# pacellie/raytracer_challenge

Measured on AMD Instinct MI355X. Metric: Mrays/s (unique rays: primary+shadow+reflection+refraction) at 1920x1080 depth-5, higher is better.
Workload: dtype f64

## Files before the change

### raytracer_challenge_amd/csrc/device_scene.h

```cpp
#pragma once
#include <stddef.h>
#include <stdint.h>

enum { OP_PRIM = 0, OP_GROUP = 1, OP_MESH = 2, OP_BVH = 3, OP_QUIRK = 4, OP_QGRID = 5, OP_CSG = 6, OP_CSG_END = 7 };

struct DOp {
  int32_t op, a, b, c;
  int32_t g;
  int32_t pad[3];
};

#define RTC_KOPS 12
#define RTC_KPLANES 6
struct DPlaneK {
  double row[4];
  int32_t prim;
  int32_t gcond;
  int32_t pad[2];
  double n[3];
};

struct DBvhNode {
  float lo0[3], hi0[3];
  float lo1[3], hi1[3];
// ... 168 lines not shown
  unsigned long long accel_nodes, group_tests, tri_tests, analytic_tests;
  unsigned long long knodes;
  unsigned long long kplanes;
  unsigned long long light_cells;
  unsigned long long kgroups;
  unsigned long long diag[64];
  unsigned long long nan_ts;
  unsigned long long guard;
  unsigned long long guard_claim;
  long long guard_info[8];
  unsigned long long wf_overflow;
};
#define RTC_STATS_LAUNCH_BYTES offsetof(DStats, nan_ts)

#define RTC_MAX_FUEL 16

#if defined(__HIPCC__) || defined(RTC_EMU)
#define RTC_HD __host__ __device__
#else
#define RTC_HD
#endif
static inline RTC_HD unsigned long long rtc_mix64(unsigned long long x) {
  x ^= x >> 33; x *= 0xff51afd7ed558ccdull; x ^= x >> 33; x *= 0xc4ceb9fe1a85ec53ull; x ^= x >> 33;
  return x;
}
static inline RTC_HD unsigned long long rtc_hit_hash_base(unsigned long long t_bits, int32_t prim, int32_t push) {
  return rtc_mix64(t_bits) ^ ((((unsigned long long)(uint32_t)prim << 32) | (unsigned long long)(uint32_t)push) * 0x9E3779B97F4A7C15ull);
}
static inline RTC_HD unsigned long long rtc_hit_hash(unsigned long long base, int depth, int kind) {
  return rtc_mix64(base ^ ((unsigned long long)(((unsigned)depth << 8) | (unsigned)kind) + 1ull) * 0xD6E8FEB86659FD93ull);
}

static inline RTC_HD unsigned long long rtc_splitmix64(unsigned long long z) {
  z = (z ^ (z >> 30)) * 0xbf58476d1ce4e5b9ull; z = (z ^ (z >> 27)) * 0x94d049bb133111ebull;
  return z ^ (z >> 31);
}
static inline RTC_HD unsigned long long rtc_area_hash(int light, double x, double y, double z) {
  unsigned long long bx, by, bz;
  __builtin_memcpy(&bx, &x, 8); __builtin_memcpy(&by, &y, 8); __builtin_memcpy(&bz, &z, 8);
  return rtc_splitmix64(rtc_splitmix64(rtc_splitmix64(rtc_splitmix64((unsigned long long)(uint32_t)light) ^ bx) ^ by) ^ bz);
}
static inline RTC_HD double rtc_area_jitter(unsigned long long h, unsigned j) {
  return (double)(rtc_splitmix64(h ^ (unsigned long long)j) >> 11) * 0x1.0p-53;
}
#define RTC_ALIGHT 16
#define RTC_SLIGHT 22

#define RTC_WF_SHADE_COUNT 32
#define RTC_WF_OVERFLOW 63
#define RTC_WF_CHUNK_NEXT 64
#define RTC_WF_TOP_COUNT (64 + 32 * 8 * (RTC_MAX_FUEL + 2))
#define RTC_WF_SHADE_TOP_COUNT (RTC_WF_TOP_COUNT + 32)
#define RTC_WF_COUNTS (RTC_WF_TOP_COUNT + 64)
#ifndef RTC_WF_CHUNK
#define RTC_WF_CHUNK 64u
#endif
#define RTC_SR_PLAIN 0x40000000
#define RTC_WF_MISS (-2)
struct DWave {
  double* rq[2];
  double* h_t;
  int32_t* h_prim;
  double* h_n12;
  double* sr;
  int32_t* sr_mat;
  int32_t* sr_node;
  double* contrib;
  int32_t* child;
  uint32_t* counts;
  uint32_t cap;
  uint32_t pad;
  unsigned long long* dig;
};
static inline uint64_t dwave_bytes(uint64_t cap, int levels) {
  return cap * (uint64_t)(7 + 7 + 1 + 2 + 9 + 3 * levels) * sizeof(double) + (cap * (uint64_t)(1 + 1 + 1 + 2 * levels) + RTC_WF_COUNTS) * sizeof(int32_t);
}
static inline void dwave_carve(DWave* W, void* mem, uint64_t cap, int levels) {
  double* d = (double*)mem;
  W->rq[0] = d; d += 7 * cap;
  W->rq[1] = d; d += 7 * cap;
  W->h_t = d; d += cap;
  W->h_n12 = d; d += 2 * cap;
  W->sr = d; d += 9 * cap;
  W->contrib = d; d += 3 * (uint64_t)levels * cap;
  int32_t* q = (int32_t*)d;
  W->h_prim = q; q += cap;
  W->sr_mat = q; q += cap;
  W->sr_node = q; q += cap;
  W->child = q; q += 2 * (uint64_t)levels * cap;
  W->counts = (uint32_t*)q;
  W->cap = (uint32_t)cap;
  W->pad = 0;
  W->dig = nullptr;
}
#ifndef RTC_BVH_STACK
#define RTC_BVH_STACK 64
#endif
```

### raytracer_challenge_amd/csrc/rtc_kernels.hip

```cpp
#include <cstdio>
#include <cstdlib>
#include <utility>

#include "../../include/rtc.h"
#include "rtc_device.hpp"

#ifdef RTC_EMU
#include "rtc_feat.hip"
constexpr int RTC_VARIANTS_BUILT = 6;
#else
constexpr int RTC_VARIANTS_BUILT = RTC_N_VARIANTS;
#endif
template <int... V>
static const RtcVariantOps& rtc_ops(int v, std::integer_sequence<int, V...>) {
  static const RtcVariantOps ops[RTC_N_VARIANTS] = {rtc_variant_ops<V>()...};
  return ops[v];
}
static const RtcVariantOps& rtc_ops(int v) { return rtc_ops(v, std::make_integer_sequence<int, RTC_VARIANTS_BUILT>{}); }
static int rtc_variant(const DScene& S, bool wavefront) {
  return rtc_pick_variant(rtc_scene_feat(S), S.n_kops > 0, S.has_area != 0, S.has_uv != 0, S.has_spot != 0, wavefront);
}

#ifndef RTC_WF_SHADE_WAVES
#define RTC_WF_SHADE_WAVES 4
// ... 138 lines not shown
    }
    if (!PIPE || n_waves != 8)
#endif
    if (threadIdx.x == 0) {
      unsigned t[4] = {0u, 0u, 0u, 0u}, b[4];
      for (int k = 0; k < 5; k++)
        for (int w = 0; w < n_waves; w++) t[end_of[k]] += s_cnt[8 * k + w];
      const int row[4] = {RTC_WF_SHADE_COUNT + level, RTC_WF_SHADE_TOP_COUNT + level, level + 1, RTC_WF_TOP_COUNT + level + 1};
      for (int e = 0; e < 4; e++) {
        const unsigned old = t[e] ? atomicAdd(&W.counts[row[e]], t[e]) : 0u;
        const bool fits = (unsigned long long)old + t[e] <= W.cap;
        if (!fits) { W.counts[RTC_WF_OVERFLOW] = 1u; stats->wf_overflow = 1ull; }
        b[e] = (e & 1) ? (fits ? W.cap - old - t[e] : W.cap) : old;
      }
      for (int k = 0; k < 5; k++)
        for (int w = 0; w < n_waves; w++) { const unsigned r = s_cnt[8 * k + w]; s_cnt[8 * k + w] = b[end_of[k]]; b[end_of[k]] += r; }
    }
    __syncthreads();
    const unsigned s = on_plane ? s_cnt[wave] + (unsigned)__popcll(m_rec0 & lt) : s_cnt[8 + wave] + (unsigned)__popcll(m_rec1 & lt);
    const unsigned jr = on_plane ? s_cnt[16 + wave] + (unsigned)__popcll(m_c0 & lt) : s_cnt[24 + wave] + (unsigned)__popcll(m_c1 & lt);
    const unsigned jt = s_cnt[32 + wave] + (unsigned)__popcll(m_c2 & lt);
    if (hit && s < W.cap) {
      double* r = W.sr;
      r[s] = st.px; r[cap + s] = st.py; r[2 * cap + s] = st.pz;
      r[3 * cap + s] = st.nx; r[4 * cap + s] = st.ny; r[5 * cap + s] = st.nz;
      if (mat >= 0) {
        r[6 * cap + s] = cr; r[7 * cap + s] = cg; r[8 * cap + s] = cbl;
        W.sr_mat[s] = mat;
      } else {
        if (!PIPE) shading_row = (int)S.mat[8 * ~mat + 7];
        W.sr_mat[s] = RTC_SR_PLAIN | shading_row;
      }
      W.sr_node[s] = (int32_t)i;
    }
    if (spawn.refl && jr < W.cap) {
      nq[jr] = st.px; nq[cap + jr] = st.py; nq[2 * cap + jr] = st.pz; nq[3 * cap + jr] = st.rx; nq[4 * cap + jr] = st.ry; nq[5 * cap + jr] = st.rz;
      nq[6 * cap + jr] = spawn.wr;
      ch[i] = (int32_t)jr;
      n_reflect++;
    }
    if (spawn.refr && jt < W.cap) {
      nq[jt] = st.ux; nq[cap + jt] = st.uy; nq[2 * cap + jt] = st.uz; nq[3 * cap + jt] = spawn.tdx; nq[4 * cap + jt] = spawn.tdy; nq[5 * cap + jt] = spawn.tdz;
      nq[6 * cap + jt] = spawn.wt;
      ch[cap + i] = (int32_t)jt;
      n_refract++;
    }
  }
  if (COUNT) {
    atomicAdd(&stats->rays_reflect, (unsigned long long)n_reflect);
    atomicAdd(&stats->rays_refract, (unsigned long long)n_refract);
  }
}

__global__ void __launch_bounds__(256) wf_gather(DCamera cam, DPixelMap pm, DWave W, unsigned n0, double* __restrict__ rgb) {
  const WorkMap wm = make_workmap(pm, cam);
  const size_t cap = W.cap;
  for (unsigned i = blockIdx.x * blockDim.x + threadIdx.x; i < n0; i += gridDim.x * blockDim.x) {
    uint64_t q;
    if (!work_to_slot(wm, i, q)) continue;
    double r = 0.0, g = 0.0, b = 0.0;
    int wait_idx[RTC_MAX_FUEL + 1];
    int wait_lvl[RTC_MAX_FUEL + 1];
    int sp = 0, lvl = 0, idx = (int)i;
    const bool digest = W.dig != nullptr && pm.digest != nullptr;
    unsigned long long dg = 0ull;
    int kind = 0;
    for (;;) {
      const double* cb = W.contrib + (size_t)lvl * 3 * cap;
      const int32_t* ch = W.child + (size_t)lvl * 2 * cap;
      const int a = ch[idx], c = ch[cap + idx];
      if (a != RTC_WF_MISS) { r += cb[idx]; g += cb[cap + idx]; b += cb[2 * cap + idx]; }
      if (digest) dg += rtc_hit_hash(W.dig[(size_t)lvl * cap + idx], lvl, kind);
      if (c >= 0) { wait_idx[sp] = c; wait_lvl[sp] = lvl + 1; sp++; }
      if (a >= 0) { idx = a; lvl++; kind = 1; continue; }
      if (sp == 0) break;
      sp--;
      idx = wait_idx[sp]; lvl = wait_lvl[sp]; kind = 2;
    }
    rgb[3 * q + 0] = r; rgb[3 * q + 1] = g; rgb[3 * q + 2] = b;
    if (digest) pm.digest[q] = dg;
  }
}


unsigned rtc_wavefront_lds_bytes(const DScene& S, bool enabled) {
#ifdef RTC_EMU
  enabled = false;
#endif
  return rtc_pick_lds_bytes(RTC_VARIANTS[rtc_variant(S, true)], enabled, rtc_lds_table_bytes(S), S.bvh_stack);
}
static RtcWfShadeBuild rtc_scene_shade_build(const DScene& S, bool count, bool level0) {
#ifdef RTC_EMU
  const bool uv = false;
#else
  const bool uv = S.has_uv != 0;
#endif
  return rtc_pick_wf_shade_build(count, uv, S.all_plain != 0, level0);
}

void rtc_kernel_info_fill(const DScene& S, bool wavefront, bool count, bool big_scene, unsigned lds_bytes, int device, rtc_kernel_info* out) {
  const int v = rtc_variant(S, wavefront);
  out->variant = v;
  out->n_kops = S.n_kops; out->n_kplanes = S.n_kplanes; out->n_kaux = 0;
  for (int i = 0; i < S.n_kops; i++) if ((S.kops[i].op == OP_BVH || S.kops[i].op == OP_MESH) && S.kops[i].pad[0] >= 0) out->n_kaux++;
  out->has_recs = S.has_recs; out->all_plain = S.all_plain; out->no_glass_mirror = S.no_glass_mirror;
  out->big_scene = big_scene ? 1 : 0;
  out->n_bvh_nodes = S.n_bvh; out->n_recs = S.n_recs; out->n_mesh_tris = S.n_mtri; out->has_mesh = S.has_mesh; out->bvh_stack = S.bvh_stack;
  out->lds_bytes = wavefront ? lds_bytes : 0u;
  out->lds_refused = 0;
#ifndef RTC_EMU
  if (wavefront && lds_bytes && rtc_ops(v).wf_ts_lds_refused && rtc_ops(v).wf_ts_lds_refused(device)) out->lds_refused = 1;
#endif
  out->trace_build = out->wf_ts_build = out->wf_shade_build0 = out->wf_shade_build = -1;
  if (wavefront) {
    out->wf_ts_build = rtc_pick_wf_ts_build(count, lds_bytes != 0);
    out->wf_shade_build0 = rtc_scene_shade_build(S, count, true);
    out->wf_shade_build = rtc_scene_shade_build(S, count, false);
  } else {
    out->trace_build = rtc_pick_trace_build(RTC_VARIANTS[v], count, big_scene, S.all_plain != 0, S.no_glass_mirror != 0);
  }
}
bool rtc_scene_is_big(unsigned long long scene_bytes) { return rtc_big_scene(scene_bytes); }

#ifndef RTC_EMU

unsigned rtc_wavefront_grid(const DScene& S, int n_cu) {
  return (unsigned)std::max(1, n_cu * rtc_ops(rtc_variant(S, true)).wf_ts_blocks_per_cu(rtc_stack_bytes(S)));
}
unsigned rtc_wavefront_lds_grid(int n_cu, int spare) { return rtc_pick_wf_ts_lds_grid(n_cu, spare); }
int rtc_wavefront_spare_cus_default(int n_cu) { return rtc_wf_spare_cus_default(n_cu); }
#endif

uint64_t rtc_wavefront_work(const DCamera& cam, const DPixelMap& pm) {
  if (pm.mode == 2 && cam.hsize >= 8 && pm.n % cam.hsize == 0) return (uint64_t)((cam.hsize + 7) / 8) * ((pm.n / cam.hsize + 7) / 8) * 64;
  return pm.n;
}

#ifndef RTC_EMU
void rtc_launch_wf_background(const DScene& S, const DCamera& cam, const DPixelMap& pm, const DWave& W, int level, unsigned n0, const DBackground& bg, unsigned blocks,
                              hipStream_t stream);
#endif
void rtc_launch_wavefront(const DScene& S, const DCamera& cam, const DPixelMap& pm, int fuel, const DWave& W, double* rgb, double* hit_t, int* hit_prim, int* hit_k,
                          DStats* stats, bool count, hipStream_t stream, unsigned blocks, unsigned shade_blocks, unsigned lds, unsigned lds_blocks, const DBackground* bg, const DBumpTable* bump) {
  if (pm.n == 0) return;
  const RtcVariantOps& ops = rtc_ops(rtc_variant(S, true));
  const RtcFrame F = {S, cam, pm, hit_t, hit_prim, hit_k, stats, stream, count};
  const unsigned n0 = (unsigned)rtc_wavefront_work(cam, pm);
  const dim3 sgrid(std::max(1u, shade_blocks)), sblock(RTC_WF_SHADE_BLOCK);
  for (int level = 0; level <= fuel + 1; level++) {
    const int tl = level <= fuel ? level : -1, sl = level - 1;
#ifndef RTC_EMU
    if (!lds || !ops.launch_wf_ts_lds(F, RtcLevel{W, tl, sl, n0, level, fuel - level, std::max(1u, lds_blocks), lds}))
#endif
    ops.launch_wf_ts(F, RtcLevel{W, tl, sl, n0, level, fuel - level, blocks, 0u});
#ifndef RTC_EMU
    if (bg && level <= fuel) rtc_launch_wf_background(S, cam, pm, W, level, n0, *bg, 4u * std::max(1u, shade_blocks), stream);
#endif
#ifndef RTC_EMU
    if (bump && level <= fuel) {
      DSceneNp N;
      static_cast<DScene&>(N) = S;
      N.bg = DBackground{0, 0};
      N.bump = *bump;
      switch (rtc_pick_wf_shade_np_build(count, S.has_uv != 0)) {
        case RTC_SH_NP_COUNT_UV: hipLaunchKernelGGL((wf_shade<true, true, true, false, false, true>), sgrid, sblock, 0, stream, N, cam, pm, W, level, n0, fuel, stats); break;
        case RTC_SH_NP_UV: hipLaunchKernelGGL((wf_shade<false, true, true, false, false, true>), sgrid, sblock, 0, stream, N, cam, pm, W, level, n0, fuel, stats); break;
        case RTC_SH_NP_COUNT: hipLaunchKernelGGL((wf_shade<true, true, false, false, false, true>), sgrid, sblock, 0, stream, N, cam, pm, W, level, n0, fuel, stats); break;
        case RTC_SH_NP: hipLaunchKernelGGL((wf_shade<false, true, false, false, false, true>), sgrid, sblock, 0, stream, N, cam, pm, W, level, n0, fuel, stats); break;
      }
    } else
#endif
    if (level <= fuel) {
      switch (rtc_scene_shade_build(S, count, level == 0)) {
#ifndef RTC_EMU
        case RTC_SH_COUNT_UV: hipLaunchKernelGGL((wf_shade<true, true, true>), sgrid, sblock, 0, stream, S, cam, pm, W, level, n0, fuel, stats); break;
        case RTC_SH_UV: hipLaunchKernelGGL((wf_shade<false, true, true>), sgrid, sblock, 0, stream, S, cam, pm, W, level, n0, fuel, stats); break;
#else
        case RTC_SH_COUNT_UV: case RTC_SH_UV: break;
#endif
        case RTC_SH_COUNT: hipLaunchKernelGGL((wf_shade<true>), sgrid, sblock, 0, stream, S, cam, pm, W, level, n0, fuel, stats); break;
        case RTC_SH_PIPE_LV0: hipLaunchKernelGGL((wf_shade<false, false, false, true, true>), sgrid, sblock, 0, stream, S, cam, pm, W, level, n0, fuel, stats); break;
        case RTC_SH_PIPE: hipLaunchKernelGGL((wf_shade<false, false, false, true, false>), sgrid, sblock, 0, stream, S, cam, pm, W, level, n0, fuel, stats); break;
        case RTC_SH_PAT: hipLaunchKernelGGL((wf_shade<false>), sgrid, sblock, 0, stream, S, cam, pm, W, level, n0, fuel, stats); break;
      }
    }
  }
  hipLaunchKernelGGL(wf_gather, dim3(std::max(1u, std::min(blocks, (n0 + 255u) / 256u))), dim3(256), 0, stream, cam, pm, W, n0, rgb);
}
void rtc_launch_wavefront(const DScene& S, const DCamera& cam, const DPixelMap& pm, int fuel, const DWave& W, double* rgb, double* hit_t, int* hit_prim, int* hit_k,
                          DStats* stats, bool count, hipStream_t stream, unsigned blocks, unsigned shade_blocks) {
  rtc_launch_wavefront(S, cam, pm, fuel, W, rgb, hit_t, hit_prim, hit_k, stats, count, stream, blocks, shade_blocks, 0u, 0u, nullptr, nullptr);
}

static dim3 rtc_elementwise_grid(unsigned long long n) { return dim3((unsigned)std::min<unsigned long long>((n + 255) / 256, 8192)); }
__global__ void __launch_bounds__(256) rtc_quantize_kernel(const double* __restrict__ rgb, unsigned char* __restrict__ out, unsigned long long n) {
  unsigned long long i = (unsigned long long)blockIdx.x * blockDim.x + threadIdx.x;
  const unsigned long long stride = (unsigned long long)gridDim.x * blockDim.x;
  for (; i < n; i += stride) {
    double x = rgb[i];
    double c = (x != x) ? 1.0 : (x < 1.0 ? x : 1.0);
    c = c > 0.0 ? c : 0.0;
    double r = round(c * 255.0);
    out[i] = (unsigned char)(r <= 0.0 ? 0.0 : (r >= 255.0 ? 255.0 : r));
  }
}
__global__ void __launch_bounds__(256) rtc_pack_hits_kernel(const double* __restrict__ t, const int* __restrict__ prim, const int* __restrict__ k, DHit* __restrict__ out, unsigned long long n) {
  for (unsigned long long i = (unsigned long long)blockIdx.x * blockDim.x + threadIdx.x; i < n; i += (unsigned long long)gridDim.x * blockDim.x) {
    DHit h;
    h.t = t[i]; h.prim = prim[i]; h.k = k[i];
    out[i] = h;
  }
}
void rtc_launch_pack_hits(const double* t, const int* prim, const int* k, DHit* out, unsigned long long n, hipStream_t stream) {
  if (n == 0) return;
  hipLaunchKernelGGL(rtc_pack_hits_kernel, rtc_elementwise_grid(n), dim3(256), 0, stream, t, prim, k, out, n);
}
void rtc_launch_quantize(const double* rgb, unsigned char* out, unsigned long long n, hipStream_t stream) {
  if (n == 0) return;
  hipLaunchKernelGGL(rtc_quantize_kernel, rtc_elementwise_grid(n), dim3(256), 0, stream, rgb, out, n);
}


template <typename T>
__global__ void __launch_bounds__(256) rtc_deinterleave_kernel(const T* __restrict__ slab, T* __restrict__ image, unsigned rowlen, unsigned vsize, unsigned n, unsigned max_rows,
                                                               unsigned band) {
  const unsigned long long total = (unsigned long long)vsize * rowlen;
  for (unsigned long long i = (unsigned long long)blockIdx.x * blockDim.x + threadIdx.x; i < total; i += (unsigned long long)gridDim.x * blockDim.x) {
    const unsigned y = (unsigned)(i / rowlen), x = (unsigned)(i % rowlen);
    const unsigned b = y / band;
    image[i] = slab[((unsigned long long)(b % n) * max_rows + (b / n) * band + y % band) * rowlen + x];
  }
}
template <typename T>
static void launch_deinterleave(const T* slab, T* image, unsigned rowlen, unsigned vsize, unsigned n, unsigned max_rows, unsigned band, hipStream_t stream) {
  const unsigned long long total = (unsigned long long)vsize * rowlen;
  if (total == 0) return;
  hipLaunchKernelGGL(rtc_deinterleave_kernel<T>, rtc_elementwise_grid(total), dim3(256), 0, stream, slab, image, rowlen, vsize, n, max_rows, band ? band : 1u);
}
void rtc_launch_deinterleave8(const unsigned char* slab, unsigned char* image, unsigned rowlen, unsigned vsize, unsigned n, unsigned max_rows, unsigned band, hipStream_t stream) {
  launch_deinterleave(slab, image, rowlen, vsize, n, max_rows, band, stream);
}
void rtc_launch_deinterleave(const double* slab, double* image, unsigned rowlen, unsigned vsize, unsigned n, unsigned max_rows, unsigned band, hipStream_t stream) {
  launch_deinterleave(slab, image, rowlen, vsize, n, max_rows, band, stream);
}
// ... 9 lines not shown
```

### raytracer_challenge_amd/csrc/rtc_scene.cpp

```cpp
#include <hip/hip_runtime_api.h>

#include <algorithm>
#include <atomic>
#include <chrono>
#include <cmath>
#include <condition_variable>
#include <cstdlib>
#include <cstdio>
#include <cstring>
#include <deque>
#include <functional>
#include <initializer_list>
#include <memory>
#include <mutex>
#include <string>
#include <thread>
#include <vector>

#include "../../include/rtc.h"
#include "adaptive_contrast.h"
#include "background_point.h"
#include "bump_normal.h"
#include "camera_sampling.h"
#include "device_scene.h"
#include "filter_weights.h"
#include "scene_build.hpp"
#include "shutter_pose.h"
#include "spot_factor.h"
#include "uv_image.h"

void rtc_launch_trace(const DScene& S, const DCamera& cam, const DPixelMap& pm, int fuel, double* rgb, double* hit_t, int* hit_prim, int* hit_k,
                      DStats* stats, bool count, hipStream_t stream, bool big_scene);
void rtc_launch_quantize(const double* rgb, unsigned char* out, unsigned long long n, hipStream_t stream);
void rtc_launch_pack_hits(const double* t, const int* prim, const int* k, DHit* out, unsigned long long n, hipStream_t stream);
void rtc_launch_deinterleave(const double* slab, double* image, unsigned rowlen, unsigned vsize, unsigned n, unsigned max_rows, unsigned band, hipStream_t stream);
void rtc_launch_deinterleave8(const unsigned char* slab, unsigned char* image, unsigned rowlen, unsigned vsize, unsigned n, unsigned max_rows, unsigned band, hipStream_t stream);
void rtc_launch_wavefront(const DScene& S, const DCamera& cam, const DPixelMap& pm, int fuel, const DWave& W, double* rgb, double* hit_t, int* hit_prim, int* hit_k,
                          DStats* stats, bool count, hipStream_t stream, unsigned blocks, unsigned shade_blocks, unsigned lds, unsigned lds_blocks, const DBackground* bg,
                          const DBumpTable* bump);
void rtc_launch_trace_np(const DScene& S, const DBumpTable& bt, const DBackground* bg, const DCamera& cam, const DPixelMap& pm, int fuel, double* rgb, double* hit_t,
                         int* hit_prim, int* hit_k, DStats* stats, bool count, hipStream_t stream);
void rtc_launch_bump_normals(const DScene& S, const DBumpTable& bt, const int32_t* prims, const double* points, const double* normals, unsigned long long n, double* out,
                             hipStream_t stream);
int rtc_bump_trace_build(const DScene& S, bool has_bg);
void rtc_launch_trace_bg(const DScene& S, const DBackground& bg, const DCamera& cam, const DPixelMap& pm, int fuel, double* rgb, double* hit_t, int* hit_prim, int* hit_k,
                         DStats* stats, bool count, hipStream_t stream);
void rtc_launch_background_colors(const DScene& S, const DBackground& bg, const double* dirs, unsigned long long n, double* rgb, hipStream_t stream);
int rtc_background_trace_build(const DScene& S);
void rtc_kernel_info_fill(const DScene& S, bool wavefront, bool count, bool big_scene, unsigned lds_bytes, int device, rtc_kernel_info* out);
bool rtc_scene_is_big(unsigned long long scene_bytes);
uint64_t rtc_wavefront_work(const DCamera& cam, const DPixelMap& pm);
unsigned rtc_wavefront_grid(const DScene& S, int n_cu);
unsigned rtc_wavefront_lds_grid(int n_cu, int spare);
int rtc_wavefront_spare_cus_default(int n_cu);
unsigned rtc_wavefront_lds_bytes(const DScene& S, bool enabled);
void rtc_launch_gen_rays(const DCamera& cam, const DPixelMap& pm, const rtc_sampling& sp, unsigned long long slot_first, unsigned long long n_slots, double* rays,
                         hipStream_t stream);
void rtc_launch_resolve_samples(const double* ray_rgb, unsigned n_samples, unsigned long long n_slots, double* dst, hipStream_t stream);
unsigned long long rtc_contrast_blocks(unsigned long long n);
unsigned long long rtc_contrast_work_words(unsigned long long n);
unsigned long long rtc_scan_work_words(unsigned long long n);
unsigned rtc_launch_scan(unsigned long long* v, unsigned long long n, unsigned long long* levels, unsigned long long* total, hipStream_t stream);
unsigned rtc_launch_contrast_compact(const double* frame, unsigned long long hsize, unsigned long long vsize, double threshold, unsigned neighbours,
                                     unsigned long long* work, unsigned long long* list, unsigned long long* count, hipStream_t stream);
void rtc_launch_resolve_samples_scatter(const double* ray_rgb, unsigned n_samples, unsigned long long n_slots, const unsigned long long* indices, double* frame,
                                        hipStream_t stream);
unsigned rtc_launch_resolve_filtered(const rtc_filter& f, const rtc_sampling& sp, unsigned long long hsize, unsigned long long row0, unsigned long long row1,
                                     unsigned long long out0, unsigned long long out1, const double* samples, double* dst, hipStream_t stream, unsigned* tile);
unsigned long long rtc_shutter_work_words(unsigned long long m);
unsigned long long* rtc_shutter_offsets(unsigned long long* work, unsigned long long m);
unsigned rtc_launch_shutter_deal(const rtc_shutter& sh, const rtc_sampling& sp, unsigned K, const DPixelMap& pm, const DCamera& cam, unsigned long long slot_first,
                                 unsigned long long m, unsigned long long* work, unsigned* order, unsigned* where, hipStream_t stream);
void rtc_launch_shutter_gen_rays(const DCamera& cam, const DPixelMap& pm, const rtc_sampling& sp, unsigned long long slot_first, const unsigned* order, unsigned off, unsigned len,
                                 unsigned m, double* rays, hipStream_t stream);
void rtc_launch_shutter_resolve(const double* ray_rgb, const unsigned* where, unsigned n_samples, unsigned long long n_slots, double* dst, hipStream_t stream);
int32_t rtc_bvh_build_device(const std::vector<bvh::Item>& items, std::vector<DBvhNode>& n2, std::vector<uint32_t>& order, uint32_t base, int leaf_max, double* frame);
int32_t rtc_bvh_build_device_keys(const std::vector<bvh::Item>& items, std::vector<DBvhNode>& n2, std::vector<uint32_t>& order, uint32_t base, int leaf_max, double* frame,
                                  std::vector<unsigned long long>* keys);

static thread_local std::string g_rtc_err;
static int rtc_fail(int code, const std::string& m) {
  g_rtc_err = m;
  return code;
}
#define HIP_OK(expr)                                                                                     \
  do {                                                                                                   \
    hipError_t e_ = (expr);                                                                              \
    if (e_ != hipSuccess) return rtc_fail(RTC_ERR_DEVICE, std::string(#expr) + ": " + hipGetErrorString(e_)); \
  } while (0)

struct rtc_scene {
  int device = 0;
// ... 3 lines not shown
  bool marker_recorded[8] = {false, false, false, false, false, false, false, false};
  std::vector<void*> allocs;
  uint64_t bytes = 0;
  DScene d{};
  bool has_bg = false;
  DBackground bg{0, 0};
  bool bg_plain = false;
  bool has_bump = false;
  uint32_t n_bumps = 0;
  DBumpTable bump{nullptr, nullptr};
  DStats* d_stats = nullptr;
  double* d_rgb = nullptr;
  double* d_hit_t = nullptr;
  int* d_hit_prim = nullptr;
  int* d_hit_k = nullptr;
  DHit* d_hits = nullptr;
  unsigned long long* d_digest = nullptr;
  unsigned long long* d_wave_dig = nullptr;
  uint64_t cap_digest = 0, cap_wave_dig = 0;
  uint8_t* d_rgb8 = nullptr;
  uint64_t cap_hits = 0, cap_rgb8 = 0;
  uint64_t* d_idx = nullptr;
  double* d_rays = nullptr;
  uint64_t cap_px = 0, cap_idx = 0, cap_rays = 0;
  double* d_srays = nullptr;
  double* d_srgb = nullptr;
  uint64_t cap_srays = 0, cap_srgb = 0;
  hipEvent_t evs0 = nullptr, evs1 = nullptr;
  unsigned long long* d_alist = nullptr;
  unsigned long long* d_awork = nullptr;
  unsigned long long* d_acount = nullptr;
  uint64_t cap_alist = 0;
  unsigned* d_shorder = nullptr;
  unsigned* d_shwhere = nullptr;
  unsigned long long* d_shwork = nullptr;
  uint64_t cap_shutter = 0;
  int kernel_version = 0;
  uint64_t tune_sig = 0;
  double tune_ms[2] = {-1.0, -1.0};
  int tune_n[2] = {0, 0};
  int tune_choice = 0;
  uint32_t n_analytic = 0;
  uint32_t n_bouncing = 0;
  uint32_t n_prims_total = 0;
  bool last_wavefront = false;
  int last_fuel = 0;
  DCsgHit* csg_slab = nullptr;
  uint64_t csg_slab_threads = 0;
  bool wave_alloc_failed = false;
  DWave wave{};
  void* wave_mem = nullptr;
  uint64_t wave_cap = 0;
  int wave_levels = 0;
  unsigned wave_blocks = 0, shade_blocks = 0;
  unsigned lds_bytes = 0;
  int n_cu = 1;
  int spare_cus = 0;
  bool counted = false;
  unsigned wave_eighths = 9;
  int bvh_depth = 0;
  int built_on_device = 0;
  uint32_t n_bvh_nodes = 0, n_mesh_tris = 0;

  template <class T>
  int upload(const std::vector<T>& v, const T** out) {
    *out = nullptr;
    if (v.empty()) return RTC_OK;
    void* p = nullptr;
    HIP_OK(hipMalloc(&p, v.size() * sizeof(T)));
    allocs.push_back(p);
    bytes += v.size() * sizeof(T);
    HIP_OK(hipMemcpy(p, v.data(), v.size() * sizeof(T), hipMemcpyHostToDevice));
    *out = (const T*)p;
    return RTC_OK;
  }
};

namespace {

struct GrowBuf { void** p; uint64_t bytes; };
int grow(uint64_t* cap, uint64_t need, std::initializer_list<GrowBuf> bufs, hipStream_t wait = nullptr) {
  if (need <= *cap) return RTC_OK;
  if (wait) HIP_OK(hipStreamSynchronize(wait));
  for (const GrowBuf& b : bufs) { (void)hipFree(*b.p); *b.p = nullptr; }
  *cap = 0;
  for (const GrowBuf& b : bufs) HIP_OK(hipMalloc(b.p, b.bytes));
  *cap = need;
  return RTC_OK;
}

int ensure_px(rtc_scene* s, uint64_t n, bool hits) {
  int rc = grow(&s->cap_px, n, {{(void**)&s->d_rgb, n * 3 * sizeof(double)}, {(void**)&s->d_hit_t, n * sizeof(double)},
                                {(void**)&s->d_hit_prim, n * sizeof(int)}, {(void**)&s->d_hit_k, n * sizeof(int)}});
  if (rc == RTC_OK && hits) rc = grow(&s->cap_hits, n, {{(void**)&s->d_hits, n * sizeof(DHit)}});
  return rc;
}
int ensure_rgb8(rtc_scene* s, uint64_t n) { return grow(&s->cap_rgb8, 3 * n, {{(void**)&s->d_rgb8, 3 * n}}); }
int ensure_rays(rtc_scene* s, uint64_t n) { return grow(&s->cap_rays, n, {{(void**)&s->d_rays, n * 6 * sizeof(double)}}); }

void pretouch_pages(void* p, size_t bytes, std::vector<std::thread>* pool) {
  if (!p || bytes < (4u << 20)) return;
  static const int T = [] { const char* e = std::getenv("RTC_PRETOUCH_THREADS"); int t = e ? std::atoi(e) : 0; return t < 0 ? 0 : (t > 32 ? 32 : t); }();
  if (T == 0) return;
  char* base = (char*)p;
  const size_t per = ((bytes / (size_t)T) + 4095) & ~(size_t)4095;
  for (int t = 0; t < T; t++) {
    const size_t b = std::min(bytes, per * (size_t)t), e = std::min(bytes, per * (size_t)(t + 1));
    if (e > b) pool->emplace_back([base, b, e] { for (size_t o = b; o < e; o += 4096) { volatile char* q = base + o; *q = 0; } });
  }
}
void join_all(std::vector<std::thread>* pool) {
  for (auto& t : *pool) t.join();
  pool->clear();
}

uint64_t wave_cap(uint64_t n_work, unsigned eighths) { return std::max<uint64_t>((n_work * eighths + 7) / 8, 4096); }
uint64_t wave_bytes(uint64_t cap, int lv) { return dwave_bytes(cap, lv); }
uint64_t wave_budget() {
  const char* e = std::getenv("RTC_WF_MAX_BYTES");
  return e ? std::strtoull(e, nullptr, 10) : (24ull << 30);
}
int ensure_wave(rtc_scene* s, uint64_t n_work, int fuel) {
  const int levels = fuel + 1;
  uint64_t cap = wave_cap(n_work, s->wave_eighths);
  if (cap > 0x7fffff00ull || wave_bytes(cap, levels) > wave_budget()) return rtc_fail(RTC_ERR_UNSUPPORTED, "launch too large for the wavefront path");
  if (cap <= s->wave_cap && levels <= s->wave_levels) return RTC_OK;
  cap = std::max(cap, s->wave_cap);
  const int lv = std::max(levels, s->wave_levels);
  HIP_OK(hipStreamSynchronize(s->stream));
  if (s->wave_mem) (void)hipFree(s->wave_mem);
  s->wave_mem = nullptr; s->wave_cap = 0; s->wave_levels = 0;
  {
    size_t free_b = 0, total_b = 0;
    if (hipMemGetInfo(&free_b, &total_b) == hipSuccess && wave_bytes(cap, lv) > (uint64_t)free_b)
      return rtc_fail(RTC_ERR_UNSUPPORTED, "the wavefront queues do not fit the device's free memory");
    const hipError_t e = std::getenv("RTC_WF_FAIL_ALLOC") ? hipErrorOutOfMemory : hipMalloc(&s->wave_mem, wave_bytes(cap, lv));
    if (e != hipSuccess) {
      (void)hipGetLastError();
      s->wave_mem = nullptr;
      if (e == hipErrorOutOfMemory) return rtc_fail(RTC_ERR_UNSUPPORTED, "hipMalloc of the wavefront queues: out of memory");
      return rtc_fail(RTC_ERR_DEVICE, std::string("hipMalloc of the wavefront queues: ") + hipGetErrorString(e));
    }
  }
  dwave_carve(&s->wave, s->wave_mem, cap, lv);
  s->wave_cap = cap;
  s->wave_levels = lv;
  return RTC_OK;
}

void to_dcam(const rtc_camera& c, DCamera* d) {
  d->hsize = c.hsize; d->vsize = c.vsize;
  d->half_width = c.half_width; d->half_height = c.half_height; d->pixel_size = c.pixel_size;
  std::memcpy(d->inv, c.transform_inv, sizeof(d->inv));
}

uint64_t launch_signature(const DCamera& cam, const DPixelMap& pm, int fuel) {
  uint64_t h = 1469598103934665603ull;
  auto mix = [&](const void* p, size_t n) { for (size_t i = 0; i < n; i++) { h ^= ((const unsigned char*)p)[i]; h *= 1099511628211ull; } };
  mix(&cam, sizeof(cam));
  mix(&pm.n, sizeof(pm.n)); mix(&pm.mode, sizeof(pm.mode)); mix(&pm.row_first, sizeof(pm.row_first)); mix(&pm.row_step, sizeof(pm.row_step)); mix(&pm.band, sizeof(pm.band));
  mix(&fuel, sizeof(fuel));
  return h ? h : 1;
}

int first_guess(const rtc_scene* s, uint64_t n_work, int fuel) {
  if (const char* e = std::getenv("RTC_FIRST_GUESS")) { const int v = std::atoi(e); if (v == 1 || v == 4) return v; }
  const bool deep = fuel >= 2 && (uint64_t)s->n_bouncing * 10u >= (uint64_t)s->n_prims_total && s->n_bouncing > 0;
  return (s->n_analytic >= 32 && deep && n_work >= (256u << 10)) ? 4 : 1;
}
int pick_path(rtc_scene* s, uint64_t sig, uint64_t n_work, int fuel, bool will_sync, bool pixel_list) {
  if (sig != s->tune_sig) { s->tune_sig = sig; s->tune_ms[0] = s->tune_ms[1] = -1.0; s->tune_n[0] = s->tune_n[1] = 0; s->tune_choice = 0; }
  if (pixel_list) return 1;
  if (s->tune_choice) return s->tune_choice;
  const int guess = first_guess(s, n_work, fuel);
  if (!will_sync) return guess;
  const int other = guess == 4 ? 1 : 4;
  const int ng = s->tune_n[guess == 4 ? 1 : 0], no = s->tune_n[other == 4 ? 1 : 0];
  return ng <= no ? guess : other;
}
void drop_wavefront(rtc_scene* s) { s->tune_ms[1] = 1e30; s->tune_n[1] = 2; s->tune_choice = 1; }
void record_sample(rtc_scene* s, bool wavefront, double ms) {
  const int k = wavefront ? 1 : 0;
  s->tune_ms[k] = s->tune_n[k] ? std::min(s->tune_ms[k], ms) : ms;
  s->tune_n[k]++;
  if (s->tune_n[0] >= 2 && s->tune_n[1] >= 2) s->tune_choice = s->tune_ms[1] < s->tune_ms[0] ? 4 : 1;
}

constexpr int RTC_LIVE_DEVICES = 64;
std::atomic<int> g_live_scenes[RTC_LIVE_DEVICES];
int live_scenes(int device) { return device >= 0 && device < RTC_LIVE_DEVICES ? g_live_scenes[device].load(std::memory_order_relaxed) : 0; }

unsigned lds_grid(const rtc_scene* s, bool will_sync) {
  const bool spare = !will_sync && live_scenes(s->device) > 1;
  return rtc_wavefront_lds_grid(s->n_cu, spare ? s->spare_cus : 0);
}

int read_clear_sticky(rtc_scene* s, DStats* h) {
  HIP_OK(hipMemcpy(h, s->d_stats, sizeof(*h), hipMemcpyDeviceToHost));
  if (h->nan_ts || h->guard || h->wf_overflow)
    HIP_OK(hipMemset((char*)s->d_stats + RTC_STATS_LAUNCH_BYTES, 0, sizeof(DStats) - RTC_STATS_LAUNCH_BYTES));
  return RTC_OK;
}

int fill_stats(rtc_scene* s, const DStats& h, uint64_t pixels, rtc_stats* stats) {
  float ms = 0.f;
  HIP_OK(hipEventElapsedTime(&ms, s->ev0, s->ev1));
  std::memset(stats, 0, sizeof(*stats));
  stats->pixels = pixels;
  stats->rays_primary = h.rays_primary; stats->rays_shadow = h.rays_shadow; stats->rays_reflect = h.rays_reflect; stats->rays_refract = h.rays_refract;
  stats->rays_container = h.rays_container; stats->accel_nodes = h.accel_nodes; stats->group_tests = h.group_tests; stats->tri_tests = h.tri_tests;
  stats->analytic_tests = h.analytic_tests; stats->nan_ts = h.nan_ts;
  stats->accel_nodes_kernarg = h.knodes; stats->analytic_tests_kernarg = h.kplanes; stats->light_grid_cells = h.light_cells;
  stats->group_tests_uniform = h.kgroups;
  stats->kernel_ms = ms;
  stats->n_launches = s->last_wavefront ? 2u * (uint32_t)s->last_fuel + 4u + (s->has_bg ? (uint32_t)s->last_fuel + 1u : 0u) : 1u;
  return RTC_OK;
}

typedef std::function<int()> AfterLaunch;
int run(rtc_scene* s, const DCamera& cam, DPixelMap pm, int fuel, double* d_rgb, bool want_hits, rtc_stats* stats, bool count, bool sync, int force = 0,
        const AfterLaunch* after = nullptr) {
  if (fuel < 0) fuel = 0;
  if (fuel > RTC_MAX_FUEL) return rtc_fail(RTC_ERR_UNSUPPORTED, "fuel exceeds RTC_MAX_FUEL (16): the reference recurses without a limit, the device keeps its pending rays per lane");
  if (s->d.n_lights == 0) fuel = 0;
  HIP_OK(hipSetDevice(s->device));
  HIP_OK(hipMemsetAsync(s->d_stats, 0, RTC_STATS_LAUNCH_BYTES, s->stream));
  HIP_OK(hipEventRecord(s->ev0, s->stream));
  const bool will_sync = sync || stats != nullptr;
  const bool tuned = force == 0 && s->kernel_version == 0;
  int path = force ? force : s->kernel_version;
  if (tuned) path = pick_path(s, launch_signature(cam, pm, fuel), rtc_wavefront_work(cam, pm), fuel, will_sync, pm.mode != 2);
  if (path == 4 && s->wave_alloc_failed && force == 0) path = 1;
  const bool wavefront = path == 4 && pm.n > 0;
  if (s->d.csg_max_hits > RTC_CSG_MAX_HITS) {
    const uint64_t threads = wavefront ? (uint64_t)s->wave_blocks * 64ull : ((rtc_wavefront_work(cam, pm) + 63) / 64) * 64;
    if (threads > s->csg_slab_threads) {
      const uint64_t bytes = threads * (uint64_t)s->d.csg_max_hits * sizeof(DCsgHit);
      const char* e = std::getenv("RTC_CSG_MAX_BYTES");
      if (bytes > (e ? std::strtoull(e, nullptr, 10) : (16ull << 30)))
        return rtc_fail(RTC_ERR_UNSUPPORTED, "the CSG intersection slab of this launch exceeds RTC_CSG_MAX_BYTES: render fewer pixels per call");
      const int rc = grow(&s->csg_slab_threads, threads, {{(void**)&s->csg_slab, bytes}}, s->stream);
      if (rc != RTC_OK) return rc;
    }
    s->d.csg_slab = s->csg_slab;
  }
  if (wavefront) {
    int rc = ensure_wave(s, rtc_wavefront_work(cam, pm), fuel);
    if (rc == RTC_ERR_UNSUPPORTED && force == 0) {
      if (tuned) drop_wavefront(s);
      else s->wave_alloc_failed = true;
      return run(s, cam, pm, fuel, d_rgb, want_hits, stats, count, sync, 1, after);
    }
    if (rc != RTC_OK) return rc;
    s->wave.dig = nullptr;
    if (pm.digest && count) {
      const uint64_t need = (uint64_t)s->wave_cap * (uint64_t)(fuel + 1);
      rc = grow(&s->cap_wave_dig, need, {{(void**)&s->d_wave_dig, need * sizeof(unsigned long long)}}, s->stream);
      if (rc != RTC_OK) return rc;
      s->wave.dig = s->d_wave_dig;
    }
    HIP_OK(hipMemsetAsync(s->wave.counts, 0, RTC_WF_COUNTS * sizeof(uint32_t), s->stream));
    HIP_OK(hipEventRecord(s->ev0, s->stream));
    rtc_launch_wavefront(s->d, cam, pm, fuel, s->wave, d_rgb, want_hits ? s->d_hit_t : nullptr, s->d_hit_prim, s->d_hit_k, s->d_stats, count, s->stream, s->wave_blocks, s->shade_blocks, s->lds_bytes,
                         lds_grid(s, will_sync), s->has_bg ? &s->bg : nullptr, s->has_bump ? &s->bump : nullptr);
  } else if (s->has_bump) {
    rtc_launch_trace_np(s->d, s->bump, s->has_bg ? &s->bg : nullptr, cam, pm, fuel, d_rgb, want_hits ? s->d_hit_t : nullptr, s->d_hit_prim, s->d_hit_k, s->d_stats, count, s->stream);
  } else if (s->has_bg) {
    rtc_launch_trace_bg(s->d, s->bg, cam, pm, fuel, d_rgb, want_hits ? s->d_hit_t : nullptr, s->d_hit_prim, s->d_hit_k, s->d_stats, count, s->stream);
  } else {
    rtc_launch_trace(s->d, cam, pm, fuel, d_rgb, want_hits ? s->d_hit_t : nullptr, s->d_hit_prim, s->d_hit_k, s->d_stats, count, s->stream, rtc_scene_is_big(s->bytes));
  }
  HIP_OK(hipGetLastError());
  HIP_OK(hipEventRecord(s->ev1, s->stream));
  s->last_wavefront = wavefront;
  s->last_fuel = fuel;
  if (after) { int rca = (*after)(); if (rca != RTC_OK) return rca; }
  if (!sync && !stats) return RTC_OK;
  HIP_OK(hipStreamSynchronize(s->stream));
  DStats h;
  int rcs = read_clear_sticky(s, &h);
  if (rcs != RTC_OK) return rcs;
  if (wavefront) {
    if (std::getenv("RTC_WF_DUMP_COUNTS")) {
      uint32_t c[64], top[64];
      HIP_OK(hipMemcpy(c, s->wave.counts, sizeof(c), hipMemcpyDeviceToHost));
      HIP_OK(hipMemcpy(top, s->wave.counts + RTC_WF_TOP_COUNT, sizeof(top), hipMemcpyDeviceToHost));
      std::fprintf(stderr, "[rtc-wf] level: rays far + near / shade records far + near:");
      for (int l = 0; l <= fuel; l++)
        std::fprintf(stderr, " %d: %u + %u / %u + %u;", l, top[l], l ? c[l] : (unsigned)rtc_wavefront_work(cam, pm), top[32 + l], c[RTC_WF_SHADE_COUNT + l]);
      std::fprintf(stderr, "\n");
    }
    uint32_t overflow = 0;
    HIP_OK(hipMemcpy(&overflow, s->wave.counts + RTC_WF_OVERFLOW, sizeof(overflow), hipMemcpyDeviceToHost));
    if (overflow) {
      const uint64_t n_work = rtc_wavefront_work(cam, pm);
      if (s->wave_eighths < 512 && wave_bytes(wave_cap(n_work, 2 * s->wave_eighths), fuel + 1) <= wave_budget() && wave_cap(n_work, 2 * s->wave_eighths) <= 0x7fffff00ull) {
        s->wave_eighths *= 2;
        const int rc2 = run(s, cam, pm, fuel, d_rgb, want_hits, stats, count, true, 4, after);
        if (rc2 != RTC_ERR_UNSUPPORTED) return rc2;
      }
      if (tuned) drop_wavefront(s);
      return run(s, cam, pm, fuel, d_rgb, want_hits, stats, count, true, 1, after);
    }
  }
  if (tuned && !count && pm.mode == 2 && !s->tune_choice) {
    float ms = 0.f;
    HIP_OK(hipEventElapsedTime(&ms, s->ev0, s->ev1));
    record_sample(s, wavefront, ms);
  }
  if (stats) {
    int rcf = fill_stats(s, h, pm.n, stats);
    if (rcf != RTC_OK) return rcf;
  }
  if (std::getenv("RTC_DIAG_DUMP")) {
    std::fprintf(stderr, "[rtc-diag]");
    for (int i = 0; i < 64; i++) std::fprintf(stderr, " %llu", (unsigned long long)h.diag[i]);
    std::fprintf(stderr, "\n");
  }
  if (h.guard) return rtc_fail(RTC_ERR_DEVICE, "traversal guard tripped (mask " + std::to_string(h.guard) + "): an index left its array; no pixel since the last check is trustworthy");
  if (h.nan_ts) return rtc_fail(RTC_ERR_NAN, "a NaN intersection t reached a sort of two or more intersections (the reference panics in Intersection::sort, src/intersection.rs:124)");
  return RTC_OK;
}

int make_pixel_map(rtc_scene* s, uint64_t hsize, uint64_t total, const uint64_t* pixel_indices, uint64_t first, uint64_t n, DPixelMap* pm, std::vector<uint64_t>* range_idx) {
  *pm = DPixelMap{};
  pm->n = n;
  if (!pixel_indices) {
    if (first % hsize == 0 && n % hsize == 0) {
      pm->mode = 2; pm->row_first = (uint32_t)(first / hsize); pm->row_step = 1;
    } else {
      range_idx->resize(n);
      for (uint64_t i = 0; i < n; i++) (*range_idx)[i] = first + i;
      pixel_indices = range_idx->data();
    }
  }
  if (pixel_indices) {
    for (uint64_t i = 0; i < n; i++)
      if (pixel_indices[i] >= total) return rtc_fail(RTC_ERR_INVALID, "pixel index exceeds the image");
    const int rc = grow(&s->cap_idx, n, {{(void**)&s->d_idx, n * sizeof(uint64_t)}});
    if (rc != RTC_OK) return rc;
    HIP_OK(hipMemcpy(s->d_idx, pixel_indices, n * sizeof(uint64_t), hipMemcpyHostToDevice));
    pm->mode = 1; pm->indices = s->d_idx;
  }
  return RTC_OK;
}
int make_pixel_map(rtc_scene* s, const rtc_camera* cam, const uint64_t* pixel_indices, uint64_t first, uint64_t n, DPixelMap* pm, std::vector<uint64_t>* range_idx) {
  return make_pixel_map(s, cam->hsize, cam->hsize * cam->vsize, pixel_indices, first, n, pm, range_idx);
}
// ... 1713 lines not shown
```

Measured before the change: 13480.

## Double-buffer wavefront counters and zero the spare set inside the gather kernel

Keeps two sets of wavefront queue counters and ping-pongs between them each frame. The final gather kernel clears the used words of the other set, so the per-frame hipMemsetAsync on the counters is usually skipped. The stats memset and the timing event records are also skipped when no sync, stats or counting is requested. This cuts stream commands between frames but adds host-side state tracking for whether each counter block is clean, which is a correctness risk if it falls out of step.

```diff
diff --git a/raytracer_challenge_amd/csrc/device_scene.h b/raytracer_challenge_amd/csrc/device_scene.h
--- a/raytracer_challenge_amd/csrc/device_scene.h
+++ b/raytracer_challenge_amd/csrc/device_scene.h
@@ -244,6 +244,7 @@
 #define RTC_WF_TOP_COUNT (64 + 32 * 8 * (RTC_MAX_FUEL + 2))
 #define RTC_WF_SHADE_TOP_COUNT (RTC_WF_TOP_COUNT + 32)
 #define RTC_WF_COUNTS (RTC_WF_TOP_COUNT + 64)
+#define RTC_WF_COUNT_BLOCKS 2
 #ifndef RTC_WF_CHUNK
 #define RTC_WF_CHUNK 64u
 #endif
@@ -265,7 +266,17 @@
   unsigned long long* dig;
 };
 static inline uint64_t dwave_bytes(uint64_t cap, int levels) {
-  return cap * (uint64_t)(7 + 7 + 1 + 2 + 9 + 3 * levels) * sizeof(double) + (cap * (uint64_t)(1 + 1 + 1 + 2 * levels) + RTC_WF_COUNTS) * sizeof(int32_t);
+  return cap * (uint64_t)(7 + 7 + 1 + 2 + 9 + 3 * levels) * sizeof(double) +
+         (cap * (uint64_t)(1 + 1 + 1 + 2 * levels) + RTC_WF_COUNT_BLOCKS * RTC_WF_COUNTS) * sizeof(int32_t);
+}
+static inline RTC_HD uint32_t rtc_wf_clean_words(uint32_t slots) { return 12u * slots + 1u; }
+static inline RTC_HD uint32_t rtc_wf_clean_word(uint32_t k, uint32_t slots) {
+  if (k < 4u * slots) {
+    const uint32_t l = k >> 2, e = k & 3u;
+    return (e == 0u ? 0u : e == 1u ? (uint32_t)RTC_WF_SHADE_COUNT : e == 2u ? (uint32_t)RTC_WF_TOP_COUNT : (uint32_t)RTC_WF_SHADE_TOP_COUNT) + l;
+  }
+  k -= 4u * slots;
+  return k < 8u * slots ? (uint32_t)RTC_WF_CHUNK_NEXT + 32u * k : (uint32_t)RTC_WF_OVERFLOW;
 }
 static inline void dwave_carve(DWave* W, void* mem, uint64_t cap, int levels) {
   double* d = (double*)mem;
diff --git a/raytracer_challenge_amd/csrc/rtc_kernels.hip b/raytracer_challenge_amd/csrc/rtc_kernels.hip
--- a/raytracer_challenge_amd/csrc/rtc_kernels.hip
+++ b/raytracer_challenge_amd/csrc/rtc_kernels.hip
@@ -214,7 +214,7 @@
   }
 }
 
-__global__ void __launch_bounds__(256) wf_gather(DCamera cam, DPixelMap pm, DWave W, unsigned n0, double* __restrict__ rgb) {
+__global__ void __launch_bounds__(256) wf_gather(DCamera cam, DPixelMap pm, DWave W, unsigned n0, double* __restrict__ rgb, uint32_t* __restrict__ clean, unsigned clean_slots) {
   const WorkMap wm = make_workmap(pm, cam);
   const size_t cap = W.cap;
   for (unsigned i = blockIdx.x * blockDim.x + threadIdx.x; i < n0; i += gridDim.x * blockDim.x) {
@@ -242,6 +242,10 @@
     rgb[3 * q + 0] = r; rgb[3 * q + 1] = g; rgb[3 * q + 2] = b;
     if (digest) pm.digest[q] = dg;
   }
+  if (clean) {
+    const unsigned n_words = rtc_wf_clean_words(clean_slots);
+    for (unsigned k = blockIdx.x * blockDim.x + threadIdx.x; k < n_words; k += gridDim.x * blockDim.x) clean[rtc_wf_clean_word(k, clean_slots)] = 0u;
+  }
 }
 
 
@@ -303,7 +307,7 @@
                               hipStream_t stream);
 #endif
 void rtc_launch_wavefront(const DScene& S, const DCamera& cam, const DPixelMap& pm, int fuel, const DWave& W, double* rgb, double* hit_t, int* hit_prim, int* hit_k,
-                          DStats* stats, bool count, hipStream_t stream, unsigned blocks, unsigned shade_blocks, unsigned lds, unsigned lds_blocks, const DBackground* bg, const DBumpTable* bump) {
+                          DStats* stats, bool count, hipStream_t stream, unsigned blocks, unsigned shade_blocks, unsigned lds, unsigned lds_blocks, const DBackground* bg, const DBumpTable* bump, uint32_t* clean) {
   if (pm.n == 0) return;
   const RtcVariantOps& ops = rtc_ops(rtc_variant(S, true));
   const RtcFrame F = {S, cam, pm, hit_t, hit_prim, hit_k, stats, stream, count};
@@ -347,11 +351,11 @@
       }
     }
   }
-  hipLaunchKernelGGL(wf_gather, dim3(std::max(1u, std::min(blocks, (n0 + 255u) / 256u))), dim3(256), 0, stream, cam, pm, W, n0, rgb);
+  hipLaunchKernelGGL(wf_gather, dim3(std::max(1u, std::min(blocks, (n0 + 255u) / 256u))), dim3(256), 0, stream, cam, pm, W, n0, rgb, clean, (unsigned)fuel + 2u);
 }
 void rtc_launch_wavefront(const DScene& S, const DCamera& cam, const DPixelMap& pm, int fuel, const DWave& W, double* rgb, double* hit_t, int* hit_prim, int* hit_k,
                           DStats* stats, bool count, hipStream_t stream, unsigned blocks, unsigned shade_blocks) {
-  rtc_launch_wavefront(S, cam, pm, fuel, W, rgb, hit_t, hit_prim, hit_k, stats, count, stream, blocks, shade_blocks, 0u, 0u, nullptr, nullptr);
+  rtc_launch_wavefront(S, cam, pm, fuel, W, rgb, hit_t, hit_prim, hit_k, stats, count, stream, blocks, shade_blocks, 0u, 0u, nullptr, nullptr, nullptr);
 }
 
 static dim3 rtc_elementwise_grid(unsigned long long n) { return dim3((unsigned)std::min<unsigned long long>((n + 255) / 256, 8192)); }
diff --git a/raytracer_challenge_amd/csrc/rtc_scene.cpp b/raytracer_challenge_amd/csrc/rtc_scene.cpp
--- a/raytracer_challenge_amd/csrc/rtc_scene.cpp
+++ b/raytracer_challenge_amd/csrc/rtc_scene.cpp
@@ -27,6 +27,7 @@
 #include "scene_build.hpp"
 #include "shutter_pose.h"
 #include "spot_factor.h"
+#include "wf_count_blocks.h"
 #include "uv_image.h"
 
 void rtc_launch_trace(const DScene& S, const DCamera& cam, const DPixelMap& pm, int fuel, double* rgb, double* hit_t, int* hit_prim, int* hit_k,
@@ -37,7 +38,7 @@
 void rtc_launch_deinterleave8(const unsigned char* slab, unsigned char* image, unsigned rowlen, unsigned vsize, unsigned n, unsigned max_rows, unsigned band, hipStream_t stream);
 void rtc_launch_wavefront(const DScene& S, const DCamera& cam, const DPixelMap& pm, int fuel, const DWave& W, double* rgb, double* hit_t, int* hit_prim, int* hit_k,
                           DStats* stats, bool count, hipStream_t stream, unsigned blocks, unsigned shade_blocks, unsigned lds, unsigned lds_blocks, const DBackground* bg,
-                          const DBumpTable* bump);
+                          const DBumpTable* bump, uint32_t* clean);
 void rtc_launch_trace_np(const DScene& S, const DBumpTable& bt, const DBackground* bg, const DCamera& cam, const DPixelMap& pm, int fuel, double* rgb, double* hit_t,
                          int* hit_prim, int* hit_k, DStats* stats, bool count, hipStream_t stream);
 void rtc_launch_bump_normals(const DScene& S, const DBumpTable& bt, const int32_t* prims, const double* points, const double* normals, unsigned long long n, double* out,
@@ -147,6 +148,8 @@
   void* wave_mem = nullptr;
   uint64_t wave_cap = 0;
   int wave_levels = 0;
+  uint32_t* wave_counts = nullptr;
+  WfCountBlocks counts;
   unsigned wave_blocks = 0, shade_blocks = 0;
   unsigned lds_bytes = 0;
   int n_cu = 1;
@@ -240,6 +243,10 @@
   dwave_carve(&s->wave, s->wave_mem, cap, lv);
   s->wave_cap = cap;
   s->wave_levels = lv;
+  s->wave_counts = s->wave.counts;
+  s->counts.dirty();
+  HIP_OK(hipMemsetAsync(s->wave_counts, 0, (size_t)RTC_WF_COUNT_BLOCKS * RTC_WF_COUNTS * sizeof(uint32_t), s->stream));
+  s->counts.zeroed();
   return RTC_OK;
 }
 
@@ -273,7 +280,7 @@
   const int ng = s->tune_n[guess == 4 ? 1 : 0], no = s->tune_n[other == 4 ? 1 : 0];
   return ng <= no ? guess : other;
 }
-void drop_wavefront(rtc_scene* s) { s->tune_ms[1] = 1e30; s->tune_n[1] = 2; s->tune_choice = 1; }
+void drop_wavefront(rtc_scene* s) { s->tune_ms[1] = 1e30; s->tune_n[1] = 2; s->tune_choice = 1; s->counts.dirty(); }
 void record_sample(rtc_scene* s, bool wavefront, double ms) {
   const int k = wavefront ? 1 : 0;
   s->tune_ms[k] = s->tune_n[k] ? std::min(s->tune_ms[k], ms) : ms;
@@ -319,14 +326,19 @@
   if (fuel > RTC_MAX_FUEL) return rtc_fail(RTC_ERR_UNSUPPORTED, "fuel exceeds RTC_MAX_FUEL (16): the reference recurses without a limit, the device keeps its pending rays per lane");
   if (s->d.n_lights == 0) fuel = 0;
   HIP_OK(hipSetDevice(s->device));
-  HIP_OK(hipMemsetAsync(s->d_stats, 0, RTC_STATS_LAUNCH_BYTES, s->stream));
-  HIP_OK(hipEventRecord(s->ev0, s->stream));
   const bool will_sync = sync || stats != nullptr;
   const bool tuned = force == 0 && s->kernel_version == 0;
   int path = force ? force : s->kernel_version;
   if (tuned) path = pick_path(s, launch_signature(cam, pm, fuel), rtc_wavefront_work(cam, pm), fuel, will_sync, pm.mode != 2);
   if (path == 4 && s->wave_alloc_failed && force == 0) path = 1;
   const bool wavefront = path == 4 && pm.n > 0;
+#ifdef RTC_DIAG
+  const bool zero_head = true;
+#else
+  const bool zero_head = count || stats != nullptr || !wavefront;
+#endif
+  if (zero_head) HIP_OK(hipMemsetAsync(s->d_stats, 0, RTC_STATS_LAUNCH_BYTES, s->stream));
+  const bool timed = will_sync || count || !wavefront;
   if (s->d.csg_max_hits > RTC_CSG_MAX_HITS) {
     const uint64_t threads = wavefront ? (uint64_t)s->wave_blocks * 64ull : ((rtc_wavefront_work(cam, pm) + 63) / 64) * 64;
     if (threads > s->csg_slab_threads) {
@@ -354,22 +366,31 @@
       if (rc != RTC_OK) return rc;
       s->wave.dig = s->d_wave_dig;
     }
-    HIP_OK(hipMemsetAsync(s->wave.counts, 0, RTC_WF_COUNTS * sizeof(uint32_t), s->stream));
-    HIP_OK(hipEventRecord(s->ev0, s->stream));
+    bool zero_counts = false;
+    const unsigned p = s->counts.begin(fuel, &zero_counts);
+    s->wave.counts = s->wave_counts + (size_t)p * RTC_WF_COUNTS;
+    if (zero_counts) HIP_OK(hipMemsetAsync(s->wave.counts, 0, RTC_WF_COUNTS * sizeof(uint32_t), s->stream));
+    if (timed) HIP_OK(hipEventRecord(s->ev0, s->stream));
     rtc_launch_wavefront(s->d, cam, pm, fuel, s->wave, d_rgb, want_hits ? s->d_hit_t : nullptr, s->d_hit_prim, s->d_hit_k, s->d_stats, count, s->stream, s->wave_blocks, s->shade_blocks, s->lds_bytes,
-                         lds_grid(s, will_sync), s->has_bg ? &s->bg : nullptr, s->has_bump ? &s->bump : nullptr);
-  } else if (s->has_bump) {
-    rtc_launch_trace_np(s->d, s->bump, s->has_bg ? &s->bg : nullptr, cam, pm, fuel, d_rgb, want_hits ? s->d_hit_t : nullptr, s->d_hit_prim, s->d_hit_k, s->d_stats, count, s->stream);
-  } else if (s->has_bg) {
-    rtc_launch_trace_bg(s->d, s->bg, cam, pm, fuel, d_rgb, want_hits ? s->d_hit_t : nullptr, s->d_hit_prim, s->d_hit_k, s->d_stats, count, s->stream);
+                         lds_grid(s, will_sync), s->has_bg ? &s->bg : nullptr, s->has_bump ? &s->bump : nullptr, s->wave_counts + (size_t)(p ^ 1u) * RTC_WF_COUNTS);
+    HIP_OK(hipGetLastError());
+    s->counts.queued(p);
   } else {
-    rtc_launch_trace(s->d, cam, pm, fuel, d_rgb, want_hits ? s->d_hit_t : nullptr, s->d_hit_prim, s->d_hit_k, s->d_stats, count, s->stream, rtc_scene_is_big(s->bytes));
-  }
-  HIP_OK(hipGetLastError());
-  HIP_OK(hipEventRecord(s->ev1, s->stream));
+    s->counts.dirty();
+    if (timed) HIP_OK(hipEventRecord(s->ev0, s->stream));
+    if (s->has_bump) {
+      rtc_launch_trace_np(s->d, s->bump, s->has_bg ? &s->bg : nullptr, cam, pm, fuel, d_rgb, want_hits ? s->d_hit_t : nullptr, s->d_hit_prim, s->d_hit_k, s->d_stats, count, s->stream);
+    } else if (s->has_bg) {
+      rtc_launch_trace_bg(s->d, s->bg, cam, pm, fuel, d_rgb, want_hits ? s->d_hit_t : nullptr, s->d_hit_prim, s->d_hit_k, s->d_stats, count, s->stream);
+    } else {
+      rtc_launch_trace(s->d, cam, pm, fuel, d_rgb, want_hits ? s->d_hit_t : nullptr, s->d_hit_prim, s->d_hit_k, s->d_stats, count, s->stream, rtc_scene_is_big(s->bytes));
+    }
+    HIP_OK(hipGetLastError());
+  }
+  if (timed) HIP_OK(hipEventRecord(s->ev1, s->stream));
   s->last_wavefront = wavefront;
   s->last_fuel = fuel;
-  if (after) { int rca = (*after)(); if (rca != RTC_OK) return rca; }
+  if (after) { int rca = (*after)(); if (rca != RTC_OK) { s->counts.dirty(); return rca; } }
   if (!sync && !stats) return RTC_OK;
   HIP_OK(hipStreamSynchronize(s->stream));
   DStats h;
@@ -389,6 +410,7 @@
     HIP_OK(hipMemcpy(&overflow, s->wave.counts + RTC_WF_OVERFLOW, sizeof(overflow), hipMemcpyDeviceToHost));
     if (overflow) {
       const uint64_t n_work = rtc_wavefront_work(cam, pm);
+      s->counts.dirty();
       if (s->wave_eighths < 512 && wave_bytes(wave_cap(n_work, 2 * s->wave_eighths), fuel + 1) <= wave_budget() && wave_cap(n_work, 2 * s->wave_eighths) <= 0x7fffff00ull) {
         s->wave_eighths *= 2;
         const int rc2 = run(s, cam, pm, fuel, d_rgb, want_hits, stats, count, true, 4, after);
diff --git a/raytracer_challenge_amd/csrc/wf_count_blocks.h b/raytracer_challenge_amd/csrc/wf_count_blocks.h
--- /dev/null
+++ b/raytracer_challenge_amd/csrc/wf_count_blocks.h
@@ -0,0 +1,19 @@
+#pragma once
+#include "device_scene.h"
+
+struct WfCountBlocks {
+  unsigned frame = 0;
+  int clean_fuel[RTC_WF_COUNT_BLOCKS] = {-1, -1};
+  int pending = -1;
+
+  void dirty() { clean_fuel[0] = clean_fuel[1] = -1; }
+  void zeroed() { clean_fuel[0] = clean_fuel[1] = RTC_MAX_FUEL; }
+  unsigned begin(int fuel, bool* need_zero) {
+    const unsigned p = frame++ & 1u;
+    *need_zero = clean_fuel[p] < fuel;
+    pending = clean_fuel[p ^ 1u] > fuel ? clean_fuel[p ^ 1u] : fuel;
+    dirty();
+    return p;
+  }
+  void queued(unsigned p) { clean_fuel[p ^ 1u] = pending; }
+};
```

New measurement: 13520 (median of 6 runs). Within noise of the previous version (+0.2%).
